# Shuijing725/CrowdNav_Prediction_AttnGraph

Measured on AMD Instinct MI355X. Metric: env-steps/sec (sim+policy fwd) at 20 humans, higher is better.
Workload: dtype f32 (big GEMMs as bf16x3 split-precision MFMA, fp32 accumulate); 1 GPU; BASELINE configs[1]: CrowdSimVarNum-v0, 20 humans, 4096 parallel envs per GPU, HH+HR attention on, policy forward + ORCA sim step + auto-reset per step; envs_per_gpu=4096, humans=20, parallelism=dp1 (envs sharded, no rollout collective), policy_init=orthogonal, torch.manual_seed(425), sampled_actions=True, side_stream_tail=inline, dephase_steps=240

## Files before the change

### crowdnav_prediction_attngraph_amd/csrc/hh_fused.hip

```cpp
#include "hh_fused.h"
#include "row_plan.h"

#include <climits>
#include <type_traits>
#include <utility>

namespace {

typedef __bf16 bf16x8 __attribute__((ext_vector_type(8)));
typedef __bf16 bf16x4 __attribute__((ext_vector_type(4)));
typedef float f32x4 __attribute__((ext_vector_type(4)));

__device__ __forceinline__ bf16x8 ldw(const char *p)
{
    return *reinterpret_cast<const bf16x8 *>(p);
}
__device__ __forceinline__ f32x4 mfma(bf16x8 a, bf16x8 b, f32x4 c) { return __builtin_amdgcn_mfma_f32_16x16x32_bf16(a, b, c, 0, 0, 0); }

template <class F, int... I>
__device__ __forceinline__ void static_for_impl(F &&f, std::integer_sequence<int, I...>) { (f(std::integral_constant<int, I>{}), ...); }
template <int N, class F>
__device__ __forceinline__ void static_for(F &&f) { static_for_impl(f, std::make_integer_sequence<int, N>{}); }

struct Split8 { bf16x8 hi, lo; };
// ... 409 lines not shown
        HH_T(14);
    }
#pragma unroll
    for (int j = 0; j < 4; ++j) {
        const int f0 = (4 * wave + j) * 16 + 4 * g;
        const f32x4 b = *reinterpret_cast<const f32x4 *>(W.os_b + f0);
#pragma unroll
        for (int rb = 0; rb < NRB; ++rb) {
            const int row = rb * 16 + i;
            if (row < t.nrows) {
                f32x4 v = acc_os[j][rb] + b;
#pragma unroll
                for (int q = 0; q < 4; ++q) v[q] = fmaxf(v[q], 0.0f);
                __builtin_nontemporal_store(v, reinterpret_cast<f32x4 *>(out_sp + (size_t)(t.r0 + row) * 256 + f0));
            }
        }
    }
    __syncthreads();
    HH_T(15);
#ifdef HH_TIMING
    if (g_hh_tim && wave == 0 && lane == 0) {
        long long *d = g_hh_tim + (size_t)blockIdx.x * 20;
        for (int k = 0; k < 16; ++k) d[k] += tacc[k];
        d[16] += 1; d[17] += t.nrows; d[18] += NRB;
        long long *d2 = g_hh_tim + (size_t)256 * 20 + ((size_t)blockIdx.x * 4 + (t.tile_ord < 3 ? t.tile_ord : 3)) * 4;
        d2[0] += tacc[4]; d2[1] += NRB; d2[2] += 1;
    }
#endif
}
}

template <int NT>
__device__ __forceinline__ void row_offsets_prologue(int E, int H, const float *__restrict__ det, int *row_off, unsigned long long *live_total, char *lds)
{
    constexpr int NW = NT / 64;
    int *part = reinterpret_cast<int *>(lds);
    const int tid = threadIdx.x, ln = tid & 63, wv = tid >> 6;
    const int chunk = (E + NT - 1) / NT;
    const int lo = tid * chunk < E ? tid * chunk : E, hi = lo + chunk < E ? lo + chunk : E;
    int sum = 0;
    for (int e = lo; e < hi; ++e) { int nd = (int)det[e]; nd = nd < 1 ? 1 : (nd > H ? H : nd); sum += nd; }
    int incl = sum;
#pragma unroll
    for (int o = 1; o < 64; o <<= 1) {
        const int v = __shfl_up(incl, o, 64);
        if (ln >= o) incl += v;
    }
    if (ln == 63) part[wv] = incl;
    __syncthreads();
    int run = incl - sum;
    for (int w = 0; w < wv; ++w) run += part[w];
    for (int e = lo; e < hi; ++e) {
        row_off[e] = run;
        int nd = (int)det[e]; nd = nd < 1 ? 1 : (nd > H ? H : nd);
        run += nd;
    }
    if (tid == NT - 1) {
        row_off[E] = run;
        if (live_total && blockIdx.x == 0) *live_total += (unsigned long long)run;
    }
    (void)NW;
    __builtin_amdgcn_fence(__ATOMIC_RELEASE, "workgroup");
    __syncthreads();
    __builtin_amdgcn_fence(__ATOMIC_ACQUIRE, "workgroup");
}

template <int FR>
__device__ __forceinline__ TileCtx next_tile(const int *row_off, int e, int e_end, int chunk_end_row, int tile_ord, int lane)
{
    TileCtx t;
    t.tile_ord = tile_ord;
    t.e_lo = e;
    t.r0 = ld_ro(row_off + e);
    const int probe = e + 1 + lane;
    const int v = probe <= e_end ? ld_ro(row_off + probe) : INT_MAX;
    const int left = chunk_end_row - t.r0;
    const int ntile = (left + FR - 1) / FR;
    const int rows = v == INT_MAX ? INT_MAX : v - t.r0;
    const bool ok = rows <= FR && left - rows <= FR * (ntile - 1);
    const int rest = left - rows;
    int key = ok ? ((((rows + 15) >> 4) + ((rest + 15) >> 4)) << 8) + (FR - rows) : INT_MAX;
    int best = key;
#pragma unroll
    for (int o = 32; o > 0; o >>= 1) { const int x = __shfl_xor(best, o, 64); best = x < best ? x : best; }
    int n_env;
    if (best == INT_MAX) {
        n_env = __popcll(__ballot(rows <= FR));
        n_env = n_env < 1 ? 1 : n_env;
    } else {
        n_env = __ffsll(__ballot(key == best));
    }
    t.n_env = n_env;
    t.nrows = __builtin_amdgcn_readfirstlane(__shfl(v, n_env - 1, 64)) - t.r0;
    const int prev_end = __shfl(v, lane >= 1 ? lane - 1 : 0, 64);
    const int st = lane >= n_env ? INT_MAX : (lane == 0 ? 0 : prev_end - t.r0);
    int cnt = 0;
    for (int k = 0; k < n_env; ++k) cnt += lane >= __builtin_amdgcn_readlane(st, k) ? 1 : 0;
    t.my_env = lane < t.nrows ? cnt - 1 : -1;
    t.my_start = __shfl(st, cnt - 1 >= 0 ? cnt - 1 : 0, 64);
    t.my_src = 0; t.my_out = t.r0 + lane;
    return t;
}

struct PlanPre { int it, out0; };
__device__ __forceinline__ PlanPre plan_prefetch(const int32_t *plan, int E, int tile, int lane)
{
    PlanPre p;
    p.it = (plan + rp_off_items(E))[(size_t)tile * 64 + lane];
    p.out0 = (plan + rp_off_rowoff())[p.it & 0xffff];
    return p;
}
__device__ __forceinline__ TileCtx plan_tile(const PlanPre &pre, int H, int tile_ord, int lane)
{
    TileCtx t;
    const unsigned long long zero = __ballot((pre.it >> 16) == 0);
    const int cnt = zero ? __ffsll((long long)zero) - 1 : 64;
    const int it = lane < cnt ? pre.it : 0;
    const int rows = it >> 16, id = it & 0xffff;
    const int out0 = pre.out0;
    int incl = rows;
#pragma unroll
    for (int o = 1; o < 64; o <<= 1) { const int y = __shfl_up(incl, o, 64); if (lane >= o) incl += y; }
    const int st = lane < cnt ? incl - rows : INT_MAX;
    t.tile_ord = tile_ord; t.e_lo = 0; t.r0 = 0; t.n_env = cnt;
    t.nrows = __builtin_amdgcn_readfirstlane(__shfl(incl, 63, 64));
    int c = 0;
    for (int k = 0; k < cnt; ++k) c += lane >= __builtin_amdgcn_readlane(st, k) ? 1 : 0;
    const int me = c - 1 >= 0 ? c - 1 : 0;
    t.my_env = lane < t.nrows ? c - 1 : -1;
    t.my_start = __shfl(st, me, 64);
    const int off = lane - t.my_start;
    t.my_src = __shfl(id, me, 64) * H + off;
    t.my_out = __shfl(out0, me, 64) + off;
    return t;
}

__global__ __launch_bounds__(256, 1) void hh_fused_wide_kernel(int E, int H, int D, const float *__restrict__ se, const float *__restrict__ det,
                                                               int *row_off, unsigned long long *live_total, HhFusedWeights W, float *__restrict__ out_sp,
                                                               unsigned long long *stamp)
{
    const CnStampScope stamp_scope(stamp);
    extern __shared__ __attribute__((aligned(16))) char lds[];
    if (det) row_offsets_prologue<256>(E, H, det, row_off, live_total, lds);
    if (stamp && blockIdx.x == 0 && threadIdx.x == 0) stamp[1] = (unsigned long long)row_off[E];
    if (W.prio) __builtin_amdgcn_s_setprio(3);
    const int lane = threadIdx.x & 63, wave = __builtin_amdgcn_readfirstlane(threadIdx.x >> 6);
    const int total = ld_ro(row_off + E);
    int e = chunk_boundary(row_off, E, total, (int)blockIdx.x, (int)gridDim.x, lane);
    const int e_end = chunk_boundary(row_off, E, total, (int)blockIdx.x + 1, (int)gridDim.x, lane);
    if (e >= e_end) return;
    int tile_ord = 0;
    const int chunk_end_row = ld_ro(row_off + e_end);
    while (e < e_end) {
        const TileCtx t = next_tile<wide::FR>(row_off, e, e_end, chunk_end_row, tile_ord++, lane);
        const int nrb = (t.nrows + 15) >> 4;
        switch (nrb) {
        case 1: wide::tile_body<1>(t, H, D, se, W, out_sp, lds, lane, wave); break;
        case 2: wide::tile_body<2>(t, H, D, se, W, out_sp, lds, lane, wave); break;
        case 3: wide::tile_body<3>(t, H, D, se, W, out_sp, lds, lane, wave); break;
        default: wide::tile_body<4>(t, H, D, se, W, out_sp, lds, lane, wave); break;
        }
        e += t.n_env;
    }
}

namespace team {

constexpr int FR = 63;
constexpr int LDS_BYTES = 163840;
template <int RB_>
struct Layout {
    static constexpr int RB = RB_;
    static constexpr bool TURNS = RB_ == 4;
    static constexpr int X_PLANE = 16 * RB * 1024;
    static constexpr int LDS_X = 0;
    static constexpr int LDS_S = 2 * X_PLANE;
    static constexpr int H_PLANE = 2 * RB * 1024;
    static constexpr int H_BYTES = 2 * H_PLANE;
    static constexpr int TEAM_S = TURNS ? 0 : 2 * H_BYTES;
    static constexpr int E0_PLANE = 4 * RB * 1024;
    static constexpr int XCH_TEAM = 4 * 2 * RB * 1024;
    static constexpr int CTR = TURNS ? LDS_X + X_PLANE + (15 * RB + 3) * 1024 + 63 * 16 : LDS_S + 4 * H_BYTES;
    static_assert(LDS_S + (TURNS ? 2 : 4) * H_BYTES + (TURNS ? 0 : 16) <= LDS_BYTES, "layout exceeds the LDS");
};

typedef __attribute__((address_space(3))) unsigned lds_u32;

typedef int i32x4 __attribute__((ext_vector_type(4)));
struct WeightBuf {
    __amdgpu_buffer_rsrc_t rs;
    unsigned emb2, qkv, os;
};
__device__ __forceinline__ WeightBuf make_weight_buf(const HhFusedWeights &W)
{
    const char *a = (const char *)W.emb2_frag, *b = (const char *)W.qkv_frag, *c = (const char *)W.os_frag;
    const char *lo = a < b ? a : b; lo = lo < c ? lo : c;
    WeightBuf wb;
    wb.rs = __builtin_amdgcn_make_buffer_rsrc((void *)lo, 0, 0x7fffffff, 0x00020000);
    wb.emb2 = (unsigned)(a - lo); wb.qkv = (unsigned)(b - lo); wb.os = (unsigned)(c - lo);
    return wb;
}
__device__ __forceinline__ bf16x8 ldb(const WeightBuf &wb, unsigned soff, unsigned voff)
{
    return __builtin_bit_cast(bf16x8, __builtin_amdgcn_raw_buffer_load_b128(wb.rs, voff, soff, 0));
}

struct RowBuf { __amdgpu_buffer_rsrc_t rs; };
__device__ __forceinline__ RowBuf make_row_buf(float *base, int r0, int nrows, int width)
{
    RowBuf rb;
    rb.rs = __builtin_amdgcn_make_buffer_rsrc((void *)(base + (size_t)r0 * width), 0, nrows * width * 4, 0x00020000);
    return rb;
}
constexpr int TRAIN_STORE_AUX = 2;
__device__ __forceinline__ void st4(const RowBuf &b, int float_off, f32x4 v)
{
    __builtin_amdgcn_raw_buffer_store_b128(__builtin_bit_cast(i32x4, v), b.rs, float_off * 4, 0, TRAIN_STORE_AUX);
}
__device__ __forceinline__ void st1(const RowBuf &b, int float_off, float v)
{
    __builtin_amdgcn_raw_buffer_store_b32(__builtin_bit_cast(int, v), b.rs, float_off * 4, 0, TRAIN_STORE_AUX);
}

__device__ __forceinline__ void team_barrier(char *lds, int bar_off, unsigned &target, int lane)
{
    lds_u32 *ctr = (lds_u32 *)(lds + bar_off);
    target += 4;
    asm volatile("s_waitcnt lgkmcnt(0)" ::: "memory");
    if (lane == 0) __hip_atomic_fetch_add(ctr, 1u, __ATOMIC_RELAXED, __HIP_MEMORY_SCOPE_WORKGROUP);
    while ((int)(__builtin_amdgcn_readfirstlane(__hip_atomic_load(ctr, __ATOMIC_RELAXED, __HIP_MEMORY_SCOPE_WORKGROUP)) - target) < 0)
        __builtin_amdgcn_s_sleep(1);
    asm volatile("" ::: "memory");
}

__device__ __forceinline__ void wait_turn(char *lds, int ctr_off, unsigned turn)
{
    lds_u32 *done = (lds_u32 *)(lds + ctr_off + 8);
    const unsigned need = 4u * turn;
    while ((int)(__builtin_amdgcn_readfirstlane(__hip_atomic_load(done, __ATOMIC_RELAXED, __HIP_MEMORY_SCOPE_WORKGROUP)) - need) < 0)
        __builtin_amdgcn_s_sleep(1);
    asm volatile("" ::: "memory");
}
__device__ __forceinline__ void finish_turn(char *lds, int ctr_off, int lane)
{
    lds_u32 *done = (lds_u32 *)(lds + ctr_off + 8);
    asm volatile("s_waitcnt lgkmcnt(0)" ::: "memory");
    if (lane == 0) __hip_atomic_fetch_add(done, 1u, __ATOMIC_RELAXED, __HIP_MEMORY_SCOPE_WORKGROUP);
}

template <int NRB, int J0, int RB>
__device__ __forceinline__ void finish_rows(const TileCtx &t, const f32x4 (&acc)[4][NRB], const char *xch, const HhFusedWeights &W,
                                            float *__restrict__ out_sp, int lane, int wave, const f32x4 *bpre = nullptr)
{
    const int i = lane & 15, g = lane >> 4, loff = lane * 16;
#pragma unroll
    for (int jj = 0; jj < 2; ++jj) {
        const int f0 = (4 * wave + J0 + jj) * 16 + 4 * g;
        const f32x4 b = bpre ? bpre[jj] : *reinterpret_cast<const f32x4 *>(W.os_b + f0);
#pragma unroll
        for (int rb = 0; rb < NRB; ++rb) {
            const f32x4 other = *reinterpret_cast<const f32x4 *>(xch + ((wave * 2 + jj) * RB + rb) * 1024 + loff);
            const int row = rb * 16 + i;
            const int orow = __shfl(t.my_out, row, 64);
            if (row < t.nrows) {
                f32x4 v = acc[J0 + jj][rb] + other + b;
#pragma unroll
                for (int q = 0; q < 4; ++q) v[q] = fmaxf(v[q], 0.0f);
                __builtin_nontemporal_store(v, reinterpret_cast<f32x4 *>(out_sp + (size_t)orow * 256 + f0));
            }
        }
    }
}

constexpr int PF = 2;

template <int NRB, bool TRAIN>
__device__ __forceinline__ void tile_body(const TileCtx &t, int H, int D, const float *__restrict__ se, const HhFusedWeights &W, const WeightBuf &WB,
                                          float *__restrict__ out_sp, char *lds, int lane_in, int wave, int tm)
{
    using L = Layout<(NRB <= 3 ? 3 : 4)>;
    constexpr int RB = L::RB, X_PLANE = L::X_PLANE, LDS_X = L::LDS_X, LDS_S = L::LDS_S, H_PLANE = L::H_PLANE, H_BYTES = L::H_BYTES,
                  E0_PLANE = L::E0_PLANE, XCH_TEAM = L::XCH_TEAM, LDS_CTR = L::CTR;
    int lane = lane_in;
    asm volatile("" : "+v"(lane));
    const int i = lane & 15, g = lane >> 4;
    const int loff = lane * 16;
    const unsigned uoff = (unsigned)loff;
    RowBuf o_e0{}, o_x{}, o_qkv{}, o_attn{};
    if (TRAIN) {
        o_e0 = make_row_buf(W.e0_out, t.r0, t.nrows, 128); o_x = make_row_buf(W.x_out, t.r0, t.nrows, 512);
        o_qkv = make_row_buf(W.qkv_out, t.r0, t.nrows, 1536); o_attn = make_row_buf(W.attn_out, t.r0, t.nrows, 512);
    }
    constexpr int NKS = (NRB + 1) / 2;
    const int w8 = 4 * tm + wave;
    RowBuf BB;
    BB.rs = __builtin_amdgcn_make_buffer_rsrc((void *)W.qkv_b, 0, 1536 * 4, 0x00020000);
#ifdef HH_TIMING
    long long tacc[16] = {0}, tlast = clock64();
#endif

    if (w8 == 0 && lane < 4) *reinterpret_cast<unsigned *>(lds + LDS_CTR + 4 * lane) = 0u;
    unsigned bar_target = 0;
    bf16x8 wq[4][8];
    {
        const int wv = w8 >> 1, half = w8 & 1;
        const unsigned wp = WB.emb2 + (unsigned)wv * 4 * 16 * 1024;
#pragma unroll
        for (int ks = 0; ks < 4; ++ks)
#pragma unroll
            for (int j = 0; j < 4; ++j) {
                wq[ks][2 * j] = ldb(WB, wp + ((ks * 8 + half * 4 + j) * 2 + 0) * 1024, uoff);
                wq[ks][2 * j + 1] = ldb(WB, wp + ((ks * 8 + half * 4 + j) * 2 + 1) * 1024, uoff);
            }
    }
    {
        const int c0 = 32 * wave + 8 * g;
#pragma unroll
        for (int rr = 0; rr < (NRB + 1) / 2; ++rr) {
            const int rb = 2 * rr + tm;
            if (rb < NRB) {
                int row = rb * 16 + i;
                row = row < t.nrows ? row : t.nrows - 1;
                const float *xp = se + (size_t)__shfl(t.my_src, row, 64) * D;
                float v[8];
#pragma unroll
                for (int u = 0; u < 8; ++u) v[u] = W.emb0_b[c0 + u];
                for (int d = 0; d < D; ++d) {
                    const float xd = xp[d];
#pragma unroll
                    for (int u = 0; u < 8; ++u) v[u] += xd * W.emb0_w[(c0 + u) * D + d];
                }
                bf16x8 hi, lo;
#pragma unroll
                for (int u = 0; u < 8; ++u) { v[u] = fmaxf(v[u], 0.0f); __bf16 h, l; split1(v[u], h, l); hi[u] = h; lo[u] = l; }
                if (TRAIN) {
                    st4(o_e0, (rb * 16 + i) * 128 + c0, f32x4{v[0], v[1], v[2], v[3]});
                    st4(o_e0, (rb * 16 + i) * 128 + c0 + 4, f32x4{v[4], v[5], v[6], v[7]});
                }
                *reinterpret_cast<bf16x8 *>(lds + LDS_S + (wave * RB + rb) * 1024 + loff) = hi;
                *reinterpret_cast<bf16x8 *>(lds + LDS_S + E0_PLANE + (wave * RB + rb) * 1024 + loff) = lo;
            }
        }
    }
    __syncthreads();
    HH_T(0);
    {
        f32x4 acc[4][NRB];
#pragma unroll
        for (int j = 0; j < 4; ++j)
#pragma unroll
            for (int rb = 0; rb < NRB; ++rb) acc[j][rb] = f32x4{0.f, 0.f, 0.f, 0.f};
#pragma unroll
        for (int ks = 0; ks < 4; ++ks) {
            bf16x8 xh[NRB], xl[NRB];
#pragma unroll
            for (int rb = 0; rb < NRB; ++rb) {
                xh[rb] = *reinterpret_cast<const bf16x8 *>(lds + LDS_S + (ks * RB + rb) * 1024 + loff);
                xl[rb] = *reinterpret_cast<const bf16x8 *>(lds + LDS_S + E0_PLANE + (ks * RB + rb) * 1024 + loff);
            }
            __builtin_amdgcn_sched_barrier(0);
            const bf16x8 *w = wq[ks];
#pragma unroll
            for (int j = 0; j < 4; ++j)
#pragma unroll
                for (int rb = 0; rb < NRB; ++rb) acc[j][rb] = mfma(w[2 * j + 1], xh[rb], acc[j][rb]);
#pragma unroll
            for (int j = 0; j < 4; ++j)
#pragma unroll
                for (int rb = 0; rb < NRB; ++rb) acc[j][rb] = mfma(w[2 * j], xl[rb], acc[j][rb]);
#pragma unroll
            for (int j = 0; j < 4; ++j)
#pragma unroll
                for (int rb = 0; rb < NRB; ++rb) acc[j][rb] = mfma(w[2 * j], xh[rb], acc[j][rb]);
            __builtin_amdgcn_sched_barrier(0);
        }
#pragma unroll
        for (int p = 0; p < 2; ++p) {
            const int fb0 = 4 * w8 + 2 * p;
            const f32x4 ba = *reinterpret_cast<const f32x4 *>(W.emb2_b + fb0 * 16 + 4 * g);
            const f32x4 bb = *reinterpret_cast<const f32x4 *>(W.emb2_b + (fb0 + 1) * 16 + 4 * g);
            const int kx = 2 * w8 + p;
#pragma unroll
            for (int rb = 0; rb < NRB; ++rb) {
                f32x4 a = acc[2 * p][rb] + ba, b = acc[2 * p + 1][rb] + bb;
#pragma unroll
                for (int q = 0; q < 4; ++q) { a[q] = fmaxf(a[q], 0.0f); b[q] = fmaxf(b[q], 0.0f); }
                if (TRAIN) {
                    st4(o_x, (rb * 16 + i) * 512 + fb0 * 16 + 4 * g, a);
                    st4(o_x, (rb * 16 + i) * 512 + fb0 * 16 + 4 * g + 16, b);
                }
                const Split8 s = split8(a, b);
                *reinterpret_cast<bf16x8 *>(lds + LDS_X + (kx * RB + rb) * 1024 + loff) = s.hi;
                if (!(L::TURNS && rb == 3 && kx == 15 && lane == 63))
                    *reinterpret_cast<bf16x8 *>(lds + LDS_X + X_PLANE + (kx * RB + rb) * 1024 + loff) = s.lo;
            }
        }
    }
    __syncthreads();
    HH_T(1);

    unsigned vmask = 0;
    {
        const int q = 16 * wave + i;
        const int eq = __shfl(t.my_env, q, 64);
#pragma unroll
        for (int jb = 0; jb < NRB; ++jb)
#pragma unroll
            for (int r = 0; r < 4; ++r) {
                const int ek = __shfl(t.my_env, 16 * jb + 4 * g + r, 64);
                if (ek == eq && eq >= 0) vmask |= 1u << (jb * 4 + r);
            }
    }

    f32x4 acc_os[4][NRB];
#pragma unroll
    for (int j = 0; j < 4; ++j)
#pragma unroll
        for (int rb = 0; rb < NRB; ++rb) acc_os[j][rb] = f32x4{0.f, 0.f, 0.f, 0.f};

    char *const H0 = lds + LDS_S + tm * L::TEAM_S, *const H1 = H0 + H_BYTES;
    const int bar = LDS_CTR + 4 * tm;
    const int h0 = ((int)blockIdx.x >> 3) & 7;
    bf16x8 wf[PF][6];
    auto ring_prologue = [&](const int hh_) __attribute__((always_inline)) {
        const unsigned wp_ = WB.qkv + (unsigned)((((h0 + 2 * hh_ + tm) & 7) * 4 + wave) * 16) * 6 * 1024;
#pragma unroll
        for (int p = 0; p < PF - 1; ++p)
#pragma unroll
            for (int c = 0; c < 6; ++c) wf[p][c] = ldb(WB, wp_ + (p * 6 + c) * 1024, uoff);
    };
    ring_prologue(0);
#pragma unroll 1
    for (int hh = 0; hh < 4; ++hh) {
        const int h = (h0 + 2 * hh + tm) & 7;
        f32x4 aq[NRB], ak[NRB], av[NRB];
#pragma unroll
        for (int rb = 0; rb < NRB; ++rb) { aq[rb] = f32x4{0.f, 0.f, 0.f, 0.f}; ak[rb] = aq[rb]; av[rb] = aq[rb]; }
        const unsigned wp = WB.qkv + (unsigned)((h * 4 + wave) * 16) * 6 * 1024;
        f32x4 bq_pf, bk_pf; float bv_pf;
        bf16x8 xh[2][NRB], xl[2][NRB];
#pragma unroll
        for (int rb = 0; rb < NRB; ++rb) {
            xh[0][rb] = *reinterpret_cast<const bf16x8 *>(lds + LDS_X + rb * 1024 + loff);
            xl[0][rb] = *reinterpret_cast<const bf16x8 *>(lds + LDS_X + X_PLANE + rb * 1024 + loff);
        }
        static_assert(16 % PF == 0, "the ring position must be compile-time inside the unrolled group");
        auto group = [&](const int k4, auto tail_c) __attribute__((always_inline)) {
        constexpr bool TAIL = decltype(tail_c)::value;
        static_for<PF>([&](auto ku_c) __attribute__((always_inline)) {
            constexpr int ku = decltype(ku_c)::value;
            const int ks = k4 + ku;
            {
                if (!TAIL || ku == 0) {
#pragma unroll
                    for (int c = 0; c < 6; ++c) wf[(ku + PF - 1) % PF][c] = ldb(WB, wp + ((ks + PF - 1) * 6 + c) * 1024, uoff);
                }
                if (!TAIL || ku + 1 < PF) {
#pragma unroll
                    for (int rb = 0; rb < NRB; ++rb) {
                        xh[(ku + 1) & 1][rb] = *reinterpret_cast<const bf16x8 *>(lds + LDS_X + ((ks + 1) * RB + rb) * 1024 + loff);
                        xl[(ku + 1) & 1][rb] = *reinterpret_cast<const bf16x8 *>(lds + LDS_X + X_PLANE + ((ks + 1) * RB + rb) * 1024 + loff);
                    }
                }
            }
            if (TAIL && ku == PF - 1) {
                const unsigned bo = (unsigned)(h * 64 + 16 * wave) * 4, bp = (unsigned)((wave & 1) * 512 + h * 64 + 16 * (wave & ~1)) * 4;
                bq_pf = __builtin_bit_cast(f32x4, __builtin_amdgcn_raw_buffer_load_b128(BB.rs, 16u * (unsigned)g, bp, 0));
                bk_pf = __builtin_bit_cast(f32x4, __builtin_amdgcn_raw_buffer_load_b128(BB.rs, 16u * (unsigned)g, bp + 64u, 0));
                bv_pf = __builtin_bit_cast(float, __builtin_amdgcn_raw_buffer_load_b32(BB.rs, 4u * (unsigned)i, bo + 4096u, 0));
            }
            const bf16x8 *w6 = wf[ku];
            const bf16x8 *xhc = xh[ku & 1], *xlc = xl[ku & 1];
#pragma unroll
            for (int rb = 0; rb < NRB; ++rb) {
                aq[rb] = mfma(w6[1], xhc[rb], aq[rb]);
                ak[rb] = mfma(w6[3], xhc[rb], ak[rb]);
                av[rb] = mfma(xhc[rb], w6[5], av[rb]);
            }
#pragma unroll
            for (int rb = 0; rb < NRB; ++rb) {
                aq[rb] = mfma(w6[0], xlc[rb], aq[rb]);
                ak[rb] = mfma(w6[2], xlc[rb], ak[rb]);
                av[rb] = mfma(xlc[rb], w6[4], av[rb]);
            }
#pragma unroll
            for (int rb = 0; rb < NRB; ++rb) {
                aq[rb] = mfma(w6[0], xhc[rb], aq[rb]);
                ak[rb] = mfma(w6[2], xhc[rb], ak[rb]);
                av[rb] = mfma(xhc[rb], w6[4], av[rb]);
            }
            constexpr int NM = 9 * NRB, ND = !TAIL || ku + 1 < PF ? 2 * NRB : 0, NV = !TAIL || ku == 0 ? 6 : (ku == PF - 1 ? 3 : 0);
            constexpr int A = NM >= 12 + ND ? 2 : 1;
            constexpr int B = (NM - NV * A) / (ND ? ND : 1);
#pragma unroll
            for (int v = 0; v < NV; ++v) {
                __builtin_amdgcn_sched_group_barrier(0x008, A, 0);
                __builtin_amdgcn_sched_group_barrier(0x020, 1, 0);
            }
#pragma unroll
            for (int d = 0; d < ND; ++d) {
                __builtin_amdgcn_sched_group_barrier(0x008, B, 0);
                __builtin_amdgcn_sched_group_barrier(0x100, 1, 0);
            }
            __builtin_amdgcn_sched_group_barrier(0x008, NM - NV * A - ND * B, 0);
            __builtin_amdgcn_sched_barrier(0);
        });
        };
#pragma unroll 1
        for (int k4 = 0; k4 < 16 - PF; k4 += PF) group(k4, std::false_type{});
        group(16 - PF, std::true_type{});
        if (hh + 1 < 4) ring_prologue(hh + 1);
        HH_T(2);
        __builtin_amdgcn_s_setprio(3);
        {
            const f32x4 bq = bq_pf, bk = bk_pf;
            const float bv = bv_pf;
#pragma unroll
            for (int rb = 0; rb < NRB; ++rb) {
                aq[rb] += bq; ak[rb] += bk;
#pragma unroll
                for (int q = 0; q < 4; ++q) av[rb][q] += bv;
            }
            if (TRAIN) {
                const int c = h * 64 + 16 * wave, cp = (wave & 1) * 512 + h * 64 + 16 * (wave & ~1);
#pragma unroll
                for (int rb = 0; rb < NRB; ++rb) {
                    st4(o_qkv, (rb * 16 + i) * 1536 + cp + 4 * g, aq[rb]);
                    st4(o_qkv, (rb * 16 + i) * 1536 + cp + 16 + 4 * g, ak[rb]);
#pragma unroll
                    for (int r = 0; r < 4; ++r) st1(o_qkv, (rb * 16 + 4 * g + r) * 1536 + 1024 + c + i, av[rb][r]);
                }
            }
        }
        if (L::TURNS) wait_turn(lds, LDS_CTR, 2 * hh + tm);
        else team_barrier(lds, bar, bar_target, lane);
        HH_T(3);
#pragma unroll
        for (int rb = 0; rb < NRB; ++rb) {
            const Split8 s = split8(aq[rb], ak[rb]);
            char *const dst = ((wave & 1) ? H1 : H0) + ((wave >> 1) * RB + rb) * 1024 + loff;
            *reinterpret_cast<bf16x8 *>(dst) = s.hi;
            *reinterpret_cast<bf16x8 *>(dst + H_PLANE) = s.lo;
        }
        team_barrier(lds, bar, bar_target, lane);
        HH_T(4);
        bf16x8 wos[2][4][2];
        {
            const unsigned op = WB.os + (unsigned)((h * 4 + wave) * 2) * 8 * 1024;
#pragma unroll
            for (int ks = 0; ks < 2; ++ks)
#pragma unroll
                for (int j = 0; j < 4; ++j) {
                    wos[ks][j][0] = ldb(WB, op + ((ks * 4 + j) * 2 + 0) * 1024, uoff);
                    wos[ks][j][1] = ldb(WB, op + ((ks * 4 + j) * 2 + 1) * 1024, uoff);
                }
        }
        float p[2 * NKS][4];
#pragma unroll
        for (int jb = 0; jb < 2 * NKS; ++jb)
#pragma unroll
            for (int r = 0; r < 4; ++r) p[jb][r] = 0.0f;
        if (wave < NRB) {
            f32x4 s[NRB];
#pragma unroll
            for (int jb = 0; jb < NRB; ++jb) s[jb] = f32x4{0.f, 0.f, 0.f, 0.f};
#pragma unroll
            for (int ks = 0; ks < 2; ++ks) {
                const bf16x8 qh = *reinterpret_cast<const bf16x8 *>(H0 + (ks * RB + wave) * 1024 + loff);
                const bf16x8 ql = *reinterpret_cast<const bf16x8 *>(H0 + H_PLANE + (ks * RB + wave) * 1024 + loff);
#pragma unroll
                for (int jb = 0; jb < NRB; ++jb) {
                    const bf16x8 kh = *reinterpret_cast<const bf16x8 *>(H1 + (ks * RB + jb) * 1024 + loff);
                    const bf16x8 kl = *reinterpret_cast<const bf16x8 *>(H1 + H_PLANE + (ks * RB + jb) * 1024 + loff);
                    s[jb] = mfma(kl, qh, s[jb]);
                    s[jb] = mfma(kh, ql, s[jb]);
                    s[jb] = mfma(kh, qh, s[jb]);
                }
            }
            if (TRAIN) {
#pragma unroll
                for (int jb = 0; jb < NRB; ++jb) s[jb] *= W.qscale;
            }
            float mx = -INFINITY;
#pragma unroll
            for (int jb = 0; jb < NRB; ++jb)
#pragma unroll
                for (int r = 0; r < 4; ++r)
                    if ((vmask >> (jb * 4 + r)) & 1u) mx = fmaxf(mx, s[jb][r]);
            mx = fmaxf(mx, __shfl_xor(mx, 16, 64));
            mx = fmaxf(mx, __shfl_xor(mx, 32, 64));
            float sum = 0.0f;
#pragma unroll
            for (int jb = 0; jb < NRB; ++jb)
#pragma unroll
                for (int r = 0; r < 4; ++r) {
                    const float e = ((vmask >> (jb * 4 + r)) & 1u) ? __builtin_amdgcn_exp2f((s[jb][r] - mx) * 1.44269504088896340736f) : 0.0f;
                    p[jb][r] = e; sum += e;
                }
            sum += __shfl_xor(sum, 16, 64);
            sum += __shfl_xor(sum, 32, 64);
            const float inv = sum > 0.0f ? 1.0f / sum : 0.0f;
#pragma unroll
            for (int jb = 0; jb < NRB; ++jb)
#pragma unroll
                for (int r = 0; r < 4; ++r) p[jb][r] *= inv;
        }
        HH_T(5);
        HH_T(6);
        if (wave < NRB) {
#pragma unroll
            for (int ks = 0; ks < NKS; ++ks) {
                const Split8 sp = split8(f32x4{p[2 * ks][0], p[2 * ks][1], p[2 * ks][2], p[2 * ks][3]},
                                         f32x4{p[2 * ks + 1][0], p[2 * ks + 1][1], p[2 * ks + 1][2], p[2 * ks + 1][3]});
                *reinterpret_cast<bf16x8 *>(H0 + (ks * RB + wave) * 1024 + loff) = sp.hi;
                *reinterpret_cast<bf16x8 *>(H0 + H_PLANE + (ks * RB + wave) * 1024 + loff) = sp.lo;
            }
        }
        team_barrier(lds, bar, bar_target, lane);
        HH_T(7);
        f32x4 o[NRB];
#pragma unroll
        for (int ib = 0; ib < NRB; ++ib) o[ib] = f32x4{0.f, 0.f, 0.f, 0.f};
#pragma unroll
        for (int ks = 0; ks < NKS; ++ks) {
            const Split8 vf = split8(av[2 * ks], 2 * ks + 1 < NRB ? av[2 * ks + 1 < NRB ? 2 * ks + 1 : 0] : f32x4{0.f, 0.f, 0.f, 0.f});
#pragma unroll
            for (int ib = 0; ib < NRB; ++ib) {
                const bf16x8 ph = *reinterpret_cast<const bf16x8 *>(H0 + (ks * RB + ib) * 1024 + loff);
                const bf16x8 pl = *reinterpret_cast<const bf16x8 *>(H0 + H_PLANE + (ks * RB + ib) * 1024 + loff);
                o[ib] = mfma(vf.lo, ph, o[ib]);
                o[ib] = mfma(vf.hi, pl, o[ib]);
                o[ib] = mfma(vf.hi, ph, o[ib]);
            }
        }
#pragma unroll
        for (int ib = 0; ib < NRB; ++ib) {
            if (TRAIN) st4(o_attn, (ib * 16 + i) * 512 + h * 64 + 16 * wave + 4 * g, o[ib]);
            bf16x4 oh, ol;
#pragma unroll
            for (int q = 0; q < 4; ++q) { __bf16 a, b; split1(o[ib][q], a, b); oh[q] = a; ol[q] = b; }
            const int off = ((wave >> 1) * RB + ib) * 1024 + loff + 8 * (wave & 1);
            *reinterpret_cast<bf16x4 *>(H1 + off) = oh;
            *reinterpret_cast<bf16x4 *>(H1 + H_PLANE + off) = ol;
        }
        HH_T(8);
        team_barrier(lds, bar, bar_target, lane);
        HH_T(9);
#pragma unroll
        for (int ks = 0; ks < 2; ++ks) {
            bf16x8 oh[NRB], ol[NRB];
#pragma unroll
            for (int rb = 0; rb < NRB; ++rb) {
                oh[rb] = *reinterpret_cast<const bf16x8 *>(H1 + (ks * RB + rb) * 1024 + loff);
                ol[rb] = *reinterpret_cast<const bf16x8 *>(H1 + H_PLANE + (ks * RB + rb) * 1024 + loff);
            }
#pragma unroll
            for (int j = 0; j < 4; ++j)
#pragma unroll
                for (int rb = 0; rb < NRB; ++rb) acc_os[j][rb] = mfma(wos[ks][j][1], oh[rb], acc_os[j][rb]);
#pragma unroll
            for (int j = 0; j < 4; ++j)
#pragma unroll
                for (int rb = 0; rb < NRB; ++rb) acc_os[j][rb] = mfma(wos[ks][j][0], ol[rb], acc_os[j][rb]);
#pragma unroll
            for (int j = 0; j < 4; ++j)
#pragma unroll
                for (int rb = 0; rb < NRB; ++rb) acc_os[j][rb] = mfma(wos[ks][j][0], oh[rb], acc_os[j][rb]);
            if (L::TURNS && ks == 1) finish_turn(lds, LDS_CTR, lane);
        }
        __builtin_amdgcn_s_setprio(1);
        HH_T(10);
    }
    f32x4 bfin[2];
#pragma unroll
    for (int jj = 0; jj < 2; ++jj) bfin[jj] = *reinterpret_cast<const f32x4 *>(W.os_b + (4 * wave + 2 * tm + jj) * 16 + 4 * g);
    __syncthreads();
    HH_T(11);
    {
        char *const xch = lds + LDS_X;
        if (tm == 0) {
#pragma unroll
            for (int jj = 0; jj < 2; ++jj)
#pragma unroll
                for (int rb = 0; rb < NRB; ++rb) *reinterpret_cast<f32x4 *>(xch + ((wave * 2 + jj) * RB + rb) * 1024 + loff) = acc_os[2 + jj][rb];
        } else {
#pragma unroll
            for (int jj = 0; jj < 2; ++jj)
#pragma unroll
                for (int rb = 0; rb < NRB; ++rb) *reinterpret_cast<f32x4 *>(xch + XCH_TEAM + ((wave * 2 + jj) * RB + rb) * 1024 + loff) = acc_os[jj][rb];
        }
        __syncthreads();
        if (tm == 0) finish_rows<NRB, 0, RB>(t, acc_os, xch + XCH_TEAM, W, out_sp, lane, wave, bfin);
        else finish_rows<NRB, 2, RB>(t, acc_os, xch, W, out_sp, lane, wave, bfin);
    }
    HH_T(12);
#ifdef HH_TIMING
    if (g_hh_tim && wave == 0 && lane == 0) {
        long long *d = g_hh_tim + ((size_t)blockIdx.x * 2 + tm) * 20;
        for (int k = 0; k < 16; ++k) d[k] += tacc[k];
        d[16] += 1; d[17] += t.nrows; d[18] += NRB;
    }
#endif
}

}

template <bool TRAIN>
__global__ __launch_bounds__(512, 2) void hh_fused_kernel(int E, int H, int D, const float *__restrict__ se, const float *__restrict__ det,
                                                          int *row_off, unsigned long long *live_total, HhFusedWeights W, float *__restrict__ out_sp,
                                                          const int32_t *__restrict__ plan, unsigned long long *stamp)
{
    const CnStampScope stamp_scope(TRAIN ? nullptr : stamp);
    extern __shared__ __attribute__((aligned(16))) char lds[];
#ifdef HH_TIMING
    const long long k_c0 = clock64(), k_r0 = wall_clock64();
#endif
    bool planned = !TRAIN && det && rp_usable(plan, E, H) && plan[1] == (int)gridDim.x;
    if (planned) {
        const int32_t *pro = plan + rp_off_rowoff();
        int bad = 0;
        for (int i = (int)threadIdx.x; i < E; i += (int)blockDim.x) {
            int nd = (int)det[i]; nd = nd < 1 ? 1 : (nd > H ? H : nd);
            bad |= (pro[i + 1] - pro[i]) ^ nd;
        }
        volatile int *flag = reinterpret_cast<volatile int *>(lds);
        if (threadIdx.x == 0) *flag = 0;
        __syncthreads();
        if (__ballot(bad != 0) != 0ull && (threadIdx.x & 63) == 0) *flag = 1;
        __syncthreads();
        planned = __builtin_amdgcn_readfirstlane(*flag) == 0;
        __syncthreads();
    }
    if (det && !planned) row_offsets_prologue<512>(E, H, det, row_off, live_total, lds);
    if (!TRAIN && stamp && blockIdx.x == 0 && threadIdx.x == 0) stamp[1] = (unsigned long long)(planned ? plan[3] : row_off[E]);
#ifdef HH_TIMING
    const long long k_c1 = clock64();
#endif
    __builtin_amdgcn_s_setprio(1);
    const int lane = threadIdx.x & 63, w8 = __builtin_amdgcn_readfirstlane(threadIdx.x >> 6);
    const int wave = w8 & 3, tm = w8 >> 2;
    int e = 0, e_end = 0, chunk_end_row = 0, n_plan = 0;
    PlanPre pre{0, 0};
    if (planned) {
        if (live_total && blockIdx.x == 0 && threadIdx.x == 0) *live_total += (unsigned long long)plan[3];
        n_plan = plan[2];
        pre = plan_prefetch(plan, E, (int)blockIdx.x, lane);
        for (int i = (int)(blockIdx.x * blockDim.x + threadIdx.x); i <= E; i += (int)(gridDim.x * blockDim.x)) row_off[i] = plan[rp_off_rowoff() + i];
    } else {
        const int total = ld_ro(row_off + E);
        e = chunk_boundary(row_off, E, total, (int)blockIdx.x, (int)gridDim.x, lane);
        e_end = chunk_boundary(row_off, E, total, (int)blockIdx.x + 1, (int)gridDim.x, lane);
        if (e >= e_end) return;
        chunk_end_row = ld_ro(row_off + e_end);
    }
    int tile_ord = 0;
    const team::WeightBuf WB = team::make_weight_buf(W);
    for (;;) {
        TileCtx t;
        if (planned) {
            if (tile_ord >= n_plan) break;
            const PlanPre cur = pre;
            ++tile_ord;
            if (tile_ord < n_plan) pre = plan_prefetch(plan, E, (int)blockIdx.x + tile_ord * (int)gridDim.x, lane);
            t = plan_tile(cur, H, tile_ord - 1, lane);
            if (t.nrows == 0) continue;
        } else {
            if (e >= e_end) break;
            t = next_tile<team::FR>(row_off, e, e_end, chunk_end_row, tile_ord++, lane);
            t.my_src = (t.e_lo + t.my_env) * H + (lane - t.my_start);
            e += t.n_env;
        }
        const int nrb = (t.nrows + 15) >> 4;
        switch (nrb) {
        case 1: team::tile_body<1, TRAIN>(t, H, D, se, W, WB, out_sp, lds, lane, wave, tm); break;
        case 2: team::tile_body<2, TRAIN>(t, H, D, se, W, WB, out_sp, lds, lane, wave, tm); break;
        case 3: team::tile_body<3, TRAIN>(t, H, D, se, W, WB, out_sp, lds, lane, wave, tm); break;
        default: team::tile_body<4, TRAIN>(t, H, D, se, W, WB, out_sp, lds, lane, wave, tm); break;
        }
    }
#ifdef HH_TIMING
    if (g_hh_tim && (threadIdx.x & 255) == 0) {
        long long *d = g_hh_tim + ((size_t)blockIdx.x * 2 + (threadIdx.x >> 8)) * 20;
        d[13] += clock64() - k_c0; d[14] += wall_clock64() - k_r0; d[15] += k_c1 - k_c0;
    }
#endif
}

__device__ __forceinline__ int koff(int g, int u, bool perm) { return perm ? 16 * (u >> 2) + 4 * g + (u & 3) : 8 * g + u; }

__device__ __forceinline__ void bake_emb2(int idx, const float *__restrict__ w, __bf16 *__restrict__ out)
{
    if (idx >= 512 * 128) return;
    const int u = idx & 7, lane = (idx >> 3) & 63, j = (idx >> 9) & 7, ks = (idx >> 12) & 3, wv = idx >> 14;
    const int fb = 8 * wv + j;
    const float x = w[(size_t)(fb * 16 + (lane & 15)) * 128 + 32 * ks + koff(lane >> 4, u, false)];
    const __bf16 hi = (__bf16)x;
    const size_t base = ((((size_t)wv * 4 + ks) * 8 + j) * 2) * 512 + lane * 8 + u;
    out[base] = hi;
    out[base + 512] = (__bf16)(x - (float)hi);
}
__device__ __forceinline__ void bake_qkv(int idx, const float *__restrict__ w, __bf16 *__restrict__ out)
{
    if (idx >= 1536 * 512) return;
    const int u = idx & 7, lane = (idx >> 3) & 63;
    int rest = idx >> 9;
    const int j = rest % 3; rest /= 3;
    const int ks = rest & 15, wv = (rest >> 4) & 3, h = rest >> 6;
    const int sec = j == 2 ? 2 : (wv & 1), blk = j == 2 ? wv : (wv & ~1) + j;
    const float x = w[(size_t)(sec * 512 + h * 64 + 16 * blk + (lane & 15)) * 512 + 32 * ks + koff(lane >> 4, u, true)];
    const __bf16 hi = (__bf16)x;
    const size_t base = (((((size_t)h * 4 + wv) * 16 + ks) * 3 + j) * 2) * 512 + lane * 8 + u;
    out[base] = hi;
    out[base + 512] = (__bf16)(x - (float)hi);
}
__device__ __forceinline__ void bake_os(int idx, const float *__restrict__ w, __bf16 *__restrict__ out)
{
    if (idx >= 256 * 512) return;
    const int u = idx & 7, lane = (idx >> 3) & 63, j = (idx >> 9) & 3, ks = (idx >> 11) & 1, wv = (idx >> 12) & 3, h = idx >> 14;
    const float x = w[(size_t)((4 * wv + j) * 16 + (lane & 15)) * 512 + h * 64 + 32 * ks + koff(lane >> 4, u, true)];
    const __bf16 hi = (__bf16)x;
    const size_t base = (((((size_t)h * 4 + wv) * 2 + ks) * 4 + j) * 2) * 512 + lane * 8 + u;
    out[base] = hi;
    out[base + 512] = (__bf16)(x - (float)hi);
}

__global__ void bake_all_kernel(const float *__restrict__ emb2_w, const float *__restrict__ qkv_w, const float *__restrict__ os_w, __bf16 *__restrict__ emb2_frag,
                                __bf16 *__restrict__ qkv_frag, __bf16 *__restrict__ os_frag)
{
    constexpr int B1 = 512 * 128 / 256, B2 = B1 + 1536 * 512 / 256;
    const int b = blockIdx.x;
    if (b < B1) bake_emb2(b * 256 + (int)threadIdx.x, emb2_w, emb2_frag);
    else if (b < B2) bake_qkv((b - B1) * 256 + (int)threadIdx.x, qkv_w, qkv_frag);
    else bake_os((b - B2) * 256 + (int)threadIdx.x, os_w, os_frag);
}

}

int hh_fused_bake(const float *emb2_w, const float *qkv_w, const float *os_w, void *emb2_frag, void *qkv_frag, void *os_frag, hipStream_t st)
{
    hipLaunchKernelGGL(bake_all_kernel, dim3((512 * 128 + 1536 * 512 + 256 * 512) / 256), dim3(256), 0, st, emb2_w, qkv_w, os_w, (__bf16 *)emb2_frag, (__bf16 *)qkv_frag,
                       (__bf16 *)os_frag);
    CN_CHECK_LAUNCH();
    return CN_OK;
}

#ifdef HH_TIMING
extern "C" int cn_hh_fused_set_timing(long long *buf)
{
    CN_HIP(hipMemcpyToSymbol(HIP_SYMBOL(g_hh_tim), &buf, sizeof(buf)));
    return CN_OK;
}
#endif

int hh_fused_forward(int E, int H, int D, const float *spatial_edges, const float *det, int *row_off, unsigned long long *live_total,
                     const HhFusedWeights &w, float *out_sp, hipStream_t st, const int32_t *row_plan)
{
    unsigned long long *stamp = cn_stamp_slot(CN_K_HH_FUSED);
    static thread_local int attr_dev = -1;
    int dev = 0;
    CN_HIP(hipGetDevice(&dev));
    if (dev != attr_dev) {
        CN_HIP(hipFuncSetAttribute(reinterpret_cast<const void *>(&hh_fused_kernel<false>), hipFuncAttributeMaxDynamicSharedMemorySize, team::LDS_BYTES));
        CN_HIP(hipFuncSetAttribute(reinterpret_cast<const void *>(&hh_fused_kernel<true>), hipFuncAttributeMaxDynamicSharedMemorySize, team::LDS_BYTES));
        CN_HIP(hipFuncSetAttribute(reinterpret_cast<const void *>(&hh_fused_wide_kernel), hipFuncAttributeMaxDynamicSharedMemorySize, wide::LDS_BYTES));
        attr_dev = dev;
    }
    const int grid = rp_workgroups(E, H);
    const bool train = w.e0_out != nullptr;
    if (train) {
        CN_REQUIRE(H <= 48 && w.x_out && w.qkv_out && w.attn_out, "hh_fused_forward: the training outputs need H <= 48 and all four buffers");
        hipLaunchKernelGGL(hh_fused_kernel<true>, dim3(grid), dim3(512), team::LDS_BYTES, st, E, H, D, spatial_edges, det, row_off, live_total, w, out_sp,
                           (const int32_t *)nullptr, stamp);
    } else if (H > team::FR)
        hipLaunchKernelGGL(hh_fused_wide_kernel, dim3(grid), dim3(256), wide::LDS_BYTES, st, E, H, D, spatial_edges, det, row_off, live_total, w, out_sp, stamp);
    else
        hipLaunchKernelGGL(hh_fused_kernel<false>, dim3(grid), dim3(512), team::LDS_BYTES, st, E, H, D, spatial_edges, det, row_off, live_total, w, out_sp,
                           row_plan, stamp);
    CN_CHECK_LAUNCH();
    return CN_OK;
}
```

Baseline: 15.64 million env-steps/s.

## Batch embedding-0 row loads, vectorize for small D, overlap weight prefetch and plan prefetch

The first embedding layer now gathers all of a wave's input rows at once, with vectorized float2/float4 loads for the D==2 and D%4==0 cases, instead of a scalar per-row loop. The emb2 weight-register loads are issued in the middle of this, between scheduling barriers, so they overlap the embedding arithmetic. The first plan-tile prefetch is moved ahead of the plan validation pass so its latency hides behind that check. The inference path holds all row values in registers at once, which raises register pressure and could hurt occupancy under launch_bounds(512,2).

```diff
diff --git a/crowdnav_prediction_attngraph_amd/csrc/hh_fused.hip b/crowdnav_prediction_attngraph_amd/csrc/hh_fused.hip
--- a/crowdnav_prediction_attngraph_amd/csrc/hh_fused.hip
+++ b/crowdnav_prediction_attngraph_amd/csrc/hh_fused.hip
@@ -735,7 +735,7 @@
     if (w8 == 0 && lane < 4) *reinterpret_cast<unsigned *>(lds + LDS_CTR + 4 * lane) = 0u;
     unsigned bar_target = 0;
     bf16x8 wq[4][8];
-    {
+    auto wq_request = [&]() __attribute__((always_inline)) {
         const int wv = w8 >> 1, half = w8 & 1;
         const unsigned wp = WB.emb2 + (unsigned)wv * 4 * 16 * 1024;
 #pragma unroll
@@ -745,36 +745,104 @@
                 wq[ks][2 * j] = ldb(WB, wp + ((ks * 8 + half * 4 + j) * 2 + 0) * 1024, uoff);
                 wq[ks][2 * j + 1] = ldb(WB, wp + ((ks * 8 + half * 4 + j) * 2 + 1) * 1024, uoff);
             }
-    }
-    {
+    };
+    auto e0_rows = [&](auto rr0_c, auto nr_c) __attribute__((always_inline)) {
+        constexpr int RR0 = decltype(rr0_c)::value, NR = decltype(nr_c)::value;
         const int c0 = 32 * wave + 8 * g;
-#pragma unroll
-        for (int rr = 0; rr < (NRB + 1) / 2; ++rr) {
-            const int rb = 2 * rr + tm;
+        int src[NR];
+#pragma unroll
+        for (int rr = 0; rr < NR; ++rr) {
+            int row = (2 * (RR0 + rr) + tm) * 16 + i;
+            row = row < t.nrows ? row : t.nrows - 1;
+            src[rr] = __shfl(t.my_src, row, 64);
+        }
+        auto xp = [&](const int rr) __attribute__((always_inline)) { return se + (size_t)src[rr] * D; };
+        float v[NR][8];
+        const float *const w0 = W.emb0_w + (size_t)c0 * D;
+        const bool vec = ((reinterpret_cast<uintptr_t>(se) | reinterpret_cast<uintptr_t>(W.emb0_w) | reinterpret_cast<uintptr_t>(W.emb0_b)) & 15) == 0;
+        if (vec && D == 2) {
+            float2 x[NR];
+#pragma unroll
+            for (int rr = 0; rr < NR; ++rr) x[rr] = *reinterpret_cast<const float2 *>(xp(rr));
+            f32x4 w[4], b[2];
+#pragma unroll
+            for (int q = 0; q < 4; ++q) w[q] = *reinterpret_cast<const f32x4 *>(w0 + 4 * q);
+#pragma unroll
+            for (int q = 0; q < 2; ++q) b[q] = *reinterpret_cast<const f32x4 *>(W.emb0_b + c0 + 4 * q);
+            __builtin_amdgcn_sched_barrier(0);
+            if (RR0 == 0) wq_request();
+            __builtin_amdgcn_sched_barrier(0);
+#pragma unroll
+            for (int rr = 0; rr < NR; ++rr)
+#pragma unroll
+                for (int u = 0; u < 8; ++u) {
+                    float a = b[u >> 2][u & 3];
+                    a += x[rr].x * w[u >> 1][2 * (u & 1)];
+                    a += x[rr].y * w[u >> 1][2 * (u & 1) + 1];
+                    v[rr][u] = a;
+                }
+        } else if (vec && (D & 3) == 0) {
+            struct Chunk { f32x4 x[NR], w[8]; };
+            auto request = [&](const int d0) __attribute__((always_inline)) {
+                Chunk c;
+#pragma unroll
+                for (int rr = 0; rr < NR; ++rr) c.x[rr] = *reinterpret_cast<const f32x4 *>(xp(rr) + d0);
+#pragma unroll
+                for (int u = 0; u < 8; ++u) c.w[u] = *reinterpret_cast<const f32x4 *>(w0 + (size_t)u * D + d0);
+                return c;
+            };
+            auto consume = [&](const Chunk &c) __attribute__((always_inline)) {
+#pragma unroll
+                for (int rr = 0; rr < NR; ++rr)
+#pragma unroll
+                    for (int u = 0; u < 8; ++u)
+#pragma unroll
+                        for (int q = 0; q < 4; ++q) v[rr][u] += c.x[rr][q] * c.w[u][q];
+            };
+            const Chunk ca = request(0);
+            f32x4 b[2];
+#pragma unroll
+            for (int q = 0; q < 2; ++q) b[q] = *reinterpret_cast<const f32x4 *>(W.emb0_b + c0 + 4 * q);
+            __builtin_amdgcn_sched_barrier(0);
+            if (RR0 == 0) wq_request();
+            __builtin_amdgcn_sched_barrier(0);
+#pragma unroll
+            for (int rr = 0; rr < NR; ++rr)
+#pragma unroll
+                for (int u = 0; u < 8; ++u) v[rr][u] = b[u >> 2][u & 3];
+            consume(ca);
+            for (int d0 = 4; d0 < D; d0 += 4) consume(request(d0));
+        } else {
+            if (RR0 == 0) wq_request();
+#pragma unroll
+            for (int rr = 0; rr < NR; ++rr) {
+#pragma unroll
+                for (int u = 0; u < 8; ++u) v[rr][u] = W.emb0_b[c0 + u];
+                for (int d = 0; d < D; ++d) {
+                    const float xd = xp(rr)[d];
+#pragma unroll
+                    for (int u = 0; u < 8; ++u) v[rr][u] += xd * w0[u * D + d];
+                }
+            }
+        }
+#pragma unroll
+        for (int rr = 0; rr < NR; ++rr) {
+            const int rb = 2 * (RR0 + rr) + tm;
             if (rb < NRB) {
-                int row = rb * 16 + i;
-                row = row < t.nrows ? row : t.nrows - 1;
-                const float *xp = se + (size_t)__shfl(t.my_src, row, 64) * D;
-                float v[8];
-#pragma unroll
-                for (int u = 0; u < 8; ++u) v[u] = W.emb0_b[c0 + u];
-                for (int d = 0; d < D; ++d) {
-                    const float xd = xp[d];
-#pragma unroll
-                    for (int u = 0; u < 8; ++u) v[u] += xd * W.emb0_w[(c0 + u) * D + d];
-                }
                 bf16x8 hi, lo;
 #pragma unroll
-                for (int u = 0; u < 8; ++u) { v[u] = fmaxf(v[u], 0.0f); __bf16 h, l; split1(v[u], h, l); hi[u] = h; lo[u] = l; }
+                for (int u = 0; u < 8; ++u) { v[rr][u] = fmaxf(v[rr][u], 0.0f); __bf16 h, l; split1(v[rr][u], h, l); hi[u] = h; lo[u] = l; }
                 if (TRAIN) {
-                    st4(o_e0, (rb * 16 + i) * 128 + c0, f32x4{v[0], v[1], v[2], v[3]});
-                    st4(o_e0, (rb * 16 + i) * 128 + c0 + 4, f32x4{v[4], v[5], v[6], v[7]});
+                    st4(o_e0, (rb * 16 + i) * 128 + c0, f32x4{v[rr][0], v[rr][1], v[rr][2], v[rr][3]});
+                    st4(o_e0, (rb * 16 + i) * 128 + c0 + 4, f32x4{v[rr][4], v[rr][5], v[rr][6], v[rr][7]});
                 }
                 *reinterpret_cast<bf16x8 *>(lds + LDS_S + (wave * RB + rb) * 1024 + loff) = hi;
                 *reinterpret_cast<bf16x8 *>(lds + LDS_S + E0_PLANE + (wave * RB + rb) * 1024 + loff) = lo;
             }
         }
-    }
+    };
+    if (TRAIN) static_for<(NRB + 1) / 2>([&](auto rr_c) __attribute__((always_inline)) { e0_rows(rr_c, std::integral_constant<int, 1>{}); });
+    else e0_rows(std::integral_constant<int, 0>{}, std::integral_constant<int, (NRB + 1) / 2>{});
     __syncthreads();
     HH_T(0);
     {
@@ -1149,7 +1217,9 @@
     const long long k_c0 = clock64(), k_r0 = wall_clock64();
 #endif
     bool planned = !TRAIN && det && rp_usable(plan, E, H) && plan[1] == (int)gridDim.x;
+    PlanPre pre{0, 0};
     if (planned) {
+        pre = plan_prefetch(plan, E, (int)blockIdx.x, (int)(threadIdx.x & 63));
         const int32_t *pro = plan + rp_off_rowoff();
         int bad = 0;
         for (int i = (int)threadIdx.x; i < E; i += (int)blockDim.x) {
@@ -1173,11 +1243,9 @@
     const int lane = threadIdx.x & 63, w8 = __builtin_amdgcn_readfirstlane(threadIdx.x >> 6);
     const int wave = w8 & 3, tm = w8 >> 2;
     int e = 0, e_end = 0, chunk_end_row = 0, n_plan = 0;
-    PlanPre pre{0, 0};
     if (planned) {
         if (live_total && blockIdx.x == 0 && threadIdx.x == 0) *live_total += (unsigned long long)plan[3];
         n_plan = plan[2];
-        pre = plan_prefetch(plan, E, (int)blockIdx.x, lane);
         for (int i = (int)(blockIdx.x * blockDim.x + threadIdx.x); i <= E; i += (int)(gridDim.x * blockDim.x)) row_off[i] = plan[rp_off_rowoff() + i];
     } else {
         const int total = ld_ro(row_off + E);
```

Result: no change. 15.76 million env-steps/s (median of 6 runs) (+0.8%).
